# distributed-lab/era-boojum

Hardware: AMD Instinct MI355X
Metric: LDE+Merkle commit Goldilocks elems/s (2^22x256, LDE x4) (higher is better)
Workload: dtype u64 (Goldilocks); 1 GPU; C3: 2^22 rows x 256 cols, LDE x4, Poseidon2 cap 16; rows=4194304, cols=256, lde=4, cap=16, tree_hasher=poseidon2, parallelism=single, launch=stream

## Files before the change

### era-boojum_amd/csrc/merkle.hip

```cpp
#include <hip/hip_runtime.h>
#include "gl.hpp"
#include "poseidon2.hpp"
#include "poseidon2_quad.hpp"
#include "bj_internal.hpp"
#include "tree_hasher.hpp"

namespace bj {

constexpr int LEAF_THREADS = 256;

__device__ __forceinline__ void store_canon4(const p2::State& s, uint64_t* o) {
    uint32_t z0[4], z1[4];
    glasm::canon_x4(s.lo[0], s.hi[0], z0[0], z1[0], s.lo[1], s.hi[1], z0[1], z1[1],
                    s.lo[2], s.hi[2], z0[2], z1[2], s.lo[3], s.hi[3], z0[3], z1[3]);
#pragma unroll
    for (int i = 0; i < 4; i++) o[i] = ((uint64_t)z1[i] << 32) | z0[i];
}

__device__ __forceinline__ void store_canon4_at(const p2::State& s, int q, uint64_t* o) {
    const int b = 4 * q;
    uint32_t z0[4], z1[4];
    glasm::canon_x4(s.lo[b], s.hi[b], z0[0], z1[0], s.lo[b + 1], s.hi[b + 1], z0[1], z1[1],
                    s.lo[b + 2], s.hi[b + 2], z0[2], z1[2], s.lo[b + 3], s.hi[b + 3], z0[3], z1[3]);
#pragma unroll
    for (int i = 0; i < 4; i++) o[i] = ((uint64_t)z1[i] << 32) | z0[i];
}

__device__ __forceinline__ void load8(p2::State& s, const uint64_t* q, size_t stride, uint32_t count) {
#pragma unroll
    for (int i = 0; i < 8; i++) {
        uint64_t v = (uint32_t)i < count ? q[(size_t)i * stride] : 0;
        s.lo[i] = (uint32_t)v;
        s.hi[i] = (uint32_t)(v >> 32);
    }
}

template <bool HAS_IN, bool FINAL, bool REM>
__device__ __forceinline__ void leaf_hash_body(const uint64_t* __restrict__ src, size_t col_stride, uint32_t n_cols,
                                               size_t n_leaves, const uint64_t* cap_in, uint64_t* out) {
    const size_t L = blockIdx.x * (size_t)LEAF_THREADS + threadIdx.x;
    if (L >= n_leaves) return;
    const uint64_t* p = src + L;
    p2::State s;
#pragma unroll
    for (int i = 0; i < 12; i++) s.lo[i] = s.hi[i] = 0;
    if (HAS_IN) {
#pragma unroll
        for (int i = 0; i < 4; i++) {
            const uint64_t v = cap_in[4 * L + i];
            s.lo[8 + i] = (uint32_t)v;
            s.hi[8 + i] = (uint32_t)(v >> 32);
        }
    }
    const uint32_t full = n_cols >> 3;
    const uint32_t rem = REM ? n_cols & 7 : 0;
    uint64_t nxt[8];
    if (full > 0) {
#pragma unroll
        for (int i = 0; i < 8; i++) nxt[i] = p[(size_t)i * col_stride];
    }
    if (full > 0) {
        for (uint32_t g = 0; g + 1 < full; g++) {
#pragma unroll
            for (int i = 0; i < 8; i++) {
                s.lo[i] = (uint32_t)nxt[i];
                s.hi[i] = (uint32_t)(nxt[i] >> 32);
            }
            const uint64_t* q = p + (size_t)(g + 1) * 8 * col_stride;
#pragma unroll
            for (int i = 0; i < 8; i++) nxt[i] = q[(size_t)i * col_stride];
            p2::permute<p2::OUT_CAP>(s);
        }
#pragma unroll
        for (int i = 0; i < 8; i++) {
            s.lo[i] = (uint32_t)nxt[i];
            s.hi[i] = (uint32_t)(nxt[i] >> 32);
        }
        if (FINAL && !REM)
            p2::permute<p2::OUT_DIGEST>(s);
        else
            p2::permute<p2::OUT_CAP>(s);
    }
    if (FINAL && REM) {
        load8(s, p + (size_t)full * 8 * col_stride, col_stride, rem);
        p2::permute<p2::OUT_DIGEST>(s);
    }
    if (FINAL) store_canon4(s, out + 4 * L);
    else store_canon4_at(s, 2, out + 4 * L);
}

template <bool HAS_IN, bool FINAL, bool REM>
__global__ __launch_bounds__(LEAF_THREADS) void leaf_hash_kernel(const uint64_t* __restrict__ src,
                                                                 size_t col_stride, uint32_t n_cols,
                                                                 size_t n_leaves, const uint64_t* cap_in,
                                                                 uint64_t* out) {
    leaf_hash_body<HAS_IN, FINAL, REM>(src, col_stride, n_cols, n_leaves, cap_in, out);
}

__global__ __launch_bounds__(LEAF_THREADS) void leaf_chunk_kernel(const uint64_t* __restrict__ src,
                                                                  size_t col_stride, uint32_t n_cols,
                                                                  uint32_t log_e, size_t n_leaves,
                                                                  uint64_t* __restrict__ out) {
    const size_t L = blockIdx.x * (size_t)LEAF_THREADS + threadIdx.x;
    if (L >= n_leaves) return;
    const uint32_t E = 1u << log_e;
    const uint64_t* p = src + (L << log_e);
    p2::State s;
#pragma unroll
    for (int i = 0; i < 12; i++) s.lo[i] = s.hi[i] = 0;
    const uint32_t total = n_cols << log_e;
    uint32_t k = 0;
    for (; k + 8 < total; k += 8) {
#pragma unroll
        for (int i = 0; i < 8; i++) {
            const uint32_t e = k + i;
            const uint64_t v = p[(size_t)(e >> log_e) * col_stride + (e & (E - 1))];
            s.lo[i] = (uint32_t)v;
            s.hi[i] = (uint32_t)(v >> 32);
        }
        p2::permute<p2::OUT_CAP>(s);
    }
    if (k < total) {
#pragma unroll
        for (int i = 0; i < 8; i++) {
            const uint32_t e = k + i;
            const uint64_t v = e < total ? p[(size_t)(e >> log_e) * col_stride + (e & (E - 1))] : 0;
            s.lo[i] = (uint32_t)v;
            s.hi[i] = (uint32_t)(v >> 32);
        }
        p2::permute<p2::OUT_DIGEST>(s);
    }
    store_canon4(s, out + 4 * L);
}

struct P2Node {
    static __device__ __forceinline__ void node(const uint64_t* l, const uint64_t* r, uint64_t* o) {
        p2::State s;
#pragma unroll
        for (int i = 0; i < 4; i++) {
            s.lo[i] = (uint32_t)l[i];
            s.hi[i] = (uint32_t)(l[i] >> 32);
            s.lo[4 + i] = (uint32_t)r[i];
            s.hi[4 + i] = (uint32_t)(r[i] >> 32);
            s.lo[8 + i] = s.hi[8 + i] = 0;
        }
        p2::permute<p2::OUT_DIGEST>(s);
        store_canon4(s, o);
    }
};

__global__ __launch_bounds__(256) void node_level_q4_kernel(const uint64_t* __restrict__ prev,
                                                            uint64_t* __restrict__ next, size_t m) {
    __shared__ uint64_t rcf[8 * 12];
    const uint32_t t = threadIdx.x;
    if (t < 8 * 12) {
        const uint32_t r = t / 12, e = t % 12, row = r < 4 ? r : r + 22;
        rcf[t] = p2::RCL.lo[row][e] | (p2::RCL.hi[row][e] << 32);
    }
    __syncthreads();
    const size_t i = (blockIdx.x * (size_t)256 + t) >> 2;
    const uint32_t p = t & 3;
    if (i >= m) return;
    const p2q::Consts k = p2q::consts(p);
    const uint64_t l = prev[8 * i + p], r = prev[8 * i + 4 + p];
    uint32_t lo[3] = {(uint32_t)l, (uint32_t)r, 0}, hi[3] = {(uint32_t)(l >> 32), (uint32_t)(r >> 32), 0};
    p2q::permute(lo, hi, rcf, p, k);
    uint32_t z0, z1;
    glasm::canon_x1(lo[0], hi[0], z0, z1);
    next[4 * i + p] = ((uint64_t)z1 << 32) | z0;
}

constexpr uint32_t NODE_FUSED_THREADS = 512;
constexpr uint32_t NODE_FUSED_LOG_DIGESTS = 8;
__global__ __launch_bounds__(NODE_FUSED_THREADS) void node_levels_q4_kernel(const uint64_t* __restrict__ prev,
                                                                           uint64_t* __restrict__ out, size_t len,
                                                                           uint32_t b, uint32_t lv) {
    __shared__ uint64_t rcf[8 * 12];
    __shared__ uint64_t buf[2][(NODE_FUSED_THREADS / 4) * 4];
    const uint32_t t = threadIdx.x;
    if (t < 8 * 12) {
        const uint32_t r = t / 12, e = t % 12, row = r < 4 ? r : r + 22;
        rcf[t] = p2::RCL.lo[row][e] | (p2::RCL.hi[row][e] << 32);
    }
    __syncthreads();
    const uint32_t q = t >> 2, p = t & 3;
    const p2q::Consts k = p2q::consts(p);
    size_t base = 0, level_len = len >> 1;
    uint32_t nodes = 1u << (b - 1);
    for (uint32_t j = 0; j < lv; j++) {
        if (q < nodes) {
            uint64_t l, r;
            if (j == 0) {
                const size_t i = (size_t)blockIdx.x * nodes + q;
                l = prev[8 * i + p];
                r = prev[8 * i + 4 + p];
            } else {
                l = buf[(j - 1) & 1][8 * q + p];
                r = buf[(j - 1) & 1][8 * q + 4 + p];
            }
            uint32_t lo[3] = {(uint32_t)l, (uint32_t)r, 0}, hi[3] = {(uint32_t)(l >> 32), (uint32_t)(r >> 32), 0};
            p2q::permute(lo, hi, rcf, p, k);
            uint32_t z0, z1;
            glasm::canon_x1(lo[0], hi[0], z0, z1);
            const uint64_t z = ((uint64_t)z1 << 32) | z0;
            out[4 * (base + (size_t)blockIdx.x * nodes + q) + p] = z;
            buf[j & 1][4 * q + p] = z;
        }
        __syncthreads();
        base += level_len;
        level_len >>= 1;
        nodes >>= 1;
    }
}

__global__ __launch_bounds__(256) void permute_kernel(uint64_t* states, size_t count) {
    const size_t i = blockIdx.x * (size_t)256 + threadIdx.x;
    if (i >= count) return;
    p2::State s;
#pragma unroll
    for (int k = 0; k < 12; k++) {
        uint64_t v = states[12 * i + k];
        s.lo[k] = (uint32_t)v;
        s.hi[k] = (uint32_t)(v >> 32);
    }
    p2::permute(s);
#pragma unroll
    for (int q = 0; q < 3; q++) store_canon4_at(s, q, states + 12 * i + 4 * q);
}

hipError_t launch_leaves(const uint64_t* src, size_t col_stride, uint32_t n_cols, size_t n_leaves, uint64_t* out,
                         hipStream_t st) {
    return launch_leaves_partial(src, col_stride, n_cols, n_leaves, nullptr, out, true, st);
}

hipError_t launch_leaves_partial(const uint64_t* src, size_t col_stride, uint32_t n_cols, size_t n_leaves,
                                 const uint64_t* cap_in, uint64_t* out, bool final_, hipStream_t st) {
    if (n_leaves == 0) return hipSuccess;
    const dim3 g((unsigned)((n_leaves + LEAF_THREADS - 1) / LEAF_THREADS));
#define BJ_LEAF(IN, FIN, REM) \
    hipLaunchKernelGGL((leaf_hash_kernel<IN, FIN, REM>), g, dim3(LEAF_THREADS), 0, st, src, col_stride, n_cols, \
                       n_leaves, cap_in, out)
#define BJ_LEAF_R(IN, FIN) \
    do {                     \
        if (n_cols & 7)      \
            BJ_LEAF(IN, FIN, true); \
        else                 \
            BJ_LEAF(IN, FIN, false); \
    } while (0)
    if (cap_in) {
        if (final_) BJ_LEAF_R(true, true);
        else BJ_LEAF_R(true, false);
    } else {
        if (final_) BJ_LEAF_R(false, true);
        else BJ_LEAF_R(false, false);
    }
#undef BJ_LEAF_R
#undef BJ_LEAF
    return hipGetLastError();
}

hipError_t launch_leaves_chunked(const uint64_t* src, size_t col_stride, uint32_t n_cols, uint32_t log_e,
                                 size_t n_leaves, uint64_t* out, hipStream_t st) {
    if (n_leaves == 0) return hipSuccess;
    hipLaunchKernelGGL(leaf_chunk_kernel, dim3((unsigned)((n_leaves + LEAF_THREADS - 1) / LEAF_THREADS)),
                       dim3(LEAF_THREADS), 0, st, src, col_stride, n_cols, log_e, n_leaves, out);
    return hipGetLastError();
}

static size_t node_q4_max() { return (size_t)knobs().node_q4_max; }

hipError_t launch_nodes(const uint64_t* leaves, size_t n_leaves, uint32_t cap_size, uint64_t* nodes,
                        hipStream_t st) {
    const size_t q4max = node_q4_max();
    if (!q4max) return launch_nodes_per_lane<P2Node>(leaves, n_leaves, cap_size, nodes, 512, st);
    const uint64_t* prev = leaves;
    uint64_t* out = nodes;
    size_t len = n_leaves;
    const auto pow2 = [](size_t x) { return x && !(x & (x - 1)); };
    const bool fuse = knobs().node_fused && pow2(n_leaves) && pow2(cap_size);
    while (len > cap_size) {
        size_t m = len / 2;
        if (m <= q4max && fuse) {
            uint32_t L = 0, C = 0;
            while (((size_t)1 << L) < len) L++;
            while (((size_t)1 << C) < cap_size) C++;
            const uint32_t b = std::min(NODE_FUSED_LOG_DIGESTS, L), lv = std::min(b, L - C);
            hipLaunchKernelGGL(node_levels_q4_kernel, dim3((unsigned)(len >> b)), dim3(NODE_FUSED_THREADS), 0, st,
                               prev, out, len, b, lv);
            prev = out + 4 * (len - (len >> (lv - 1)));
            out += 4 * (len - (len >> lv));
            len >>= lv;
            continue;
        }
        if (m <= q4max)
            hipLaunchKernelGGL(node_level_q4_kernel, dim3((unsigned)((m + 63) / 64)), dim3(256), 0, st, prev, out, m);
        else
            hipLaunchKernelGGL(node_level_kernel<P2Node>, dim3((unsigned)((m + 255) / 256)), dim3(256), 0, st, prev,
                               out, m);
        prev = out;
        out += 4 * m;
        len = m;
    }
    return hipGetLastError();
}

hipError_t launch_permute(uint64_t* states, size_t count, hipStream_t st) {
    if (count == 0) return hipSuccess;
    hipLaunchKernelGGL(permute_kernel, dim3((unsigned)((count + 255) / 256)), dim3(256), 0, st, states, count);
    return hipGetLastError();
}

}
```

### era-boojum_amd/csrc/poseidon2.hpp

```cpp
#pragma once
#include "gl.hpp"
#include "gl_asm.hpp"

namespace p2 {

struct RcLimbs {
    uint64_t lo[30][12];
    uint64_t hi[30][12];
};

constexpr uint64_t RC_FLAT[30][12] = {
#include "poseidon2_rc.inc"
};

constexpr RcLimbs make_rc_limbs() {
    RcLimbs r{};
    for (int i = 0; i < 30; i++)
        for (int j = 0; j < 12; j++) {
            r.lo[i][j] = RC_FLAT[i][j] & 0xFFFFFFFFull;
            r.hi[i][j] = RC_FLAT[i][j] >> 32;
        }
    return r;
}

__device__ __constant__ static const RcLimbs RCL = make_rc_limbs();

namespace sched {
constexpr uint64_t P = 0xFFFFFFFF00000001ull;
constexpr uint64_t addm(uint64_t a, uint64_t b) { return (uint64_t)(((unsigned __int128)a + b) % P); }
constexpr uint64_t subm(uint64_t a, uint64_t b) { return addm(a, P - b % P); }
constexpr uint64_t mulm(uint64_t a, uint64_t b) { return (uint64_t)(((unsigned __int128)a * b) % P); }
constexpr int SH[12] = {4, 14, 11, 8, 0, 5, 2, 9, 13, 6, 3, 12};
constexpr uint64_t FULL_RC_BOUND = ~0ull - (1ull << 41) + 1;
constexpr uint64_t LIMB_RC_BOUND = (1ull << 63) + (1ull << 62);
struct Values {
    uint64_t k[11];
    uint64_t d[10];
    uint64_t rc26[12];
};
constexpr Values derive() {
    Values v{};
    uint64_t f[12] = {RC_FLAT[4][0]};
    for (int q = 0; q < 11; q++) {
        const int r = 4 + 2 * q;
        uint64_t s = 0;
        for (int i = 1; i < 12; i++) s = addm(s, f[i]);
        v.k[q] = subm(RC_FLAT[r + 1][0], s);
        f[0] = 0;
        for (int i = 0; i < 12; i++) f[i] = addm(addm(mulm(f[i], 1ull << SH[i]), s), v.k[q]);
        s = 0;
        for (int i = 1; i < 12; i++) s = addm(s, f[i]);
        f[0] = 0;
        for (int i = 0; i < 12; i++) f[i] = addm(mulm(f[i], 1ull << SH[i]), s);
        if (q < 10) {
            v.d[q] = subm(RC_FLAT[r + 2][0], f[0]);
            f[0] = RC_FLAT[r + 2][0];
        }
    }
    for (int i = 0; i < 12; i++) v.rc26[i] = subm(RC_FLAT[26][i], f[i]);
    return v;
}
constexpr Values V = derive();
constexpr bool full_rcs_fit() {
    for (int r : {0, 1, 2, 3, 27, 28, 29})
        for (int i = 0; i < 12; i++)
            if (RC_FLAT[r][i] >= FULL_RC_BOUND) return false;
    return RC_FLAT[4][0] < FULL_RC_BOUND;
}
static_assert(full_rcs_fit(), "a full-round constant is too large for the one-add form");

constexpr uint64_t LAZY_OFF = 2 * 0xFFFFFFFFull;
constexpr uint64_t me_row_sum(int i) { return (i & 1) ? 48 : 64; }
constexpr uint64_t lazy_off(int i) { return me_row_sum(i) * LAZY_OFF; }
constexpr uint64_t lazy_fix_lo(int i) { return 1 + 2 * me_row_sum(i); }
constexpr uint64_t lazy_fix_hi(int i) { return 0xFFFFFFFFull - 2 * me_row_sum(i); }
constexpr bool lazy_in(int r) { return (r >= 1 && r <= 3) || (r >= 27 && r <= 29); }
constexpr bool lazy_rcs_fit() {
    for (int r = 0; r < 30; r++)
        for (int i = 0; i < 12; i++)
            if ((lazy_in(r) || (r == 4 && i == 0)) &&
                (RC_FLAT[r][i] < lazy_off(i) || RC_FLAT[r][i] - lazy_off(i) >= FULL_RC_BOUND))
                return false;
    return true;
}
static_assert(lazy_rcs_fit(), "a full-round constant is smaller than the lazy offset it takes out");
static_assert((lazy_fix_lo(0) + (lazy_fix_hi(0) << 32) + lazy_off(0)) == P &&
                  (lazy_fix_lo(1) + (lazy_fix_hi(1) << 32) + lazy_off(1)) == P,
              "the two-limb form of -lazy_off");
}

struct Sched {
    uint64_t rcw8[30][8];
    uint64_t rcw4[30][4];
    uint64_t k_lo[11], k_hi[11];
    uint64_t d_lo[10], d_hi[10];
    uint64_t rc26_w[12], rc26_lo[12], rc26_hi[12];
    uint64_t rcl8[30][8];
    uint64_t rcl4[30][4];
};
constexpr Sched make_sched() {
    Sched s{};
    for (int r = 0; r < 30; r++)
        for (int i = 0; i < 12; i++) {
            (i < 8 ? s.rcw8[r][i] : s.rcw4[r][i - 8]) = RC_FLAT[r][i];
            const bool lazy = sched::lazy_in(r) || (r == 4 && i == 0);
            (i < 8 ? s.rcl8[r][i] : s.rcl4[r][i - 8]) = RC_FLAT[r][i] - (lazy ? sched::lazy_off(i) : 0);
        }
    for (int q = 0; q < 11; q++) { s.k_lo[q] = sched::V.k[q] & 0xFFFFFFFFull; s.k_hi[q] = sched::V.k[q] >> 32; }
    for (int q = 0; q < 10; q++) { s.d_lo[q] = sched::V.d[q] & 0xFFFFFFFFull; s.d_hi[q] = sched::V.d[q] >> 32; }
    for (int i = 0; i < 12; i++) {
        s.rc26_w[i] = sched::V.rc26[i];
        s.rc26_lo[i] = sched::V.rc26[i] & 0xFFFFFFFFull;
        s.rc26_hi[i] = sched::V.rc26[i] >> 32;
    }
    return s;
}
__device__ __constant__ static const Sched SCH = make_sched();

struct State {
    uint32_t lo[12], hi[12];
};

__device__ __forceinline__ void sbox_lazy_x4(const uint32_t* lo, const uint32_t* hi, uint64_t* Lin, uint64_t* Hin) {
    uint32_t a0, a1, b0, b1, c0, c1, d0, d1;
    glasm::mul_x4(lo[0], hi[0], lo[0], hi[0], a0, a1, lo[1], hi[1], lo[1], hi[1], b0, b1,
                  lo[2], hi[2], lo[2], hi[2], c0, c1, lo[3], hi[3], lo[3], hi[3], d0, d1);
    uint32_t e0, e1, f0, f1, g0, g1, h0, h1;
    glasm::mul_x4(a0, a1, lo[0], hi[0], e0, e1, b0, b1, lo[1], hi[1], f0, f1,
                  c0, c1, lo[2], hi[2], g0, g1, d0, d1, lo[3], hi[3], h0, h1);
    uint32_t i0, i1, j0, j1, k0, k1, l0, l1;
    glasm::mul_x4(a0, a1, a0, a1, i0, i1, b0, b1, b0, b1, j0, j1,
                  c0, c1, c0, c1, k0, k1, d0, d1, d0, d1, l0, l1);
    glasm::mul_lazy_x4(e0, e1, i0, i1, Lin[0], Hin[0], f0, f1, j0, j1, Lin[1], Hin[1],
                       g0, g1, k0, k1, Lin[2], Hin[2], h0, h1, l0, l1, Lin[3], Hin[3]);
}

__device__ __forceinline__ void sbox_x1(uint32_t& lo, uint32_t& hi) {
    uint32_t a0, a1, e0, e1, i0, i1;
    glasm::mul_x1(lo, hi, lo, hi, a0, a1);
    glasm::mul_x2(a0, a1, lo, hi, e0, e1, a0, a1, a0, a1, i0, i1);
    glasm::mul_x1(e0, e1, i0, i1, lo, hi);
}

__device__ __forceinline__ void m4_limbs(uint64_t& x0, uint64_t& x1, uint64_t& x2, uint64_t& x3) {
    uint64_t t0 = x0 + x1;
    uint64_t t1 = x2 + x3;
    uint64_t t2 = (x1 << 1) + t1;
    uint64_t t3 = (x3 << 1) + t0;
    uint64_t t4 = (t1 << 2) + t3;
    uint64_t t5 = (t0 << 2) + t2;
    uint64_t t6 = t3 + t5;
    uint64_t t7 = t2 + t4;
    x0 = t6; x1 = t5; x2 = t7; x3 = t4;
}

__device__ __forceinline__ uint64_t add_lo_u64(uint32_t lo, uint64_t b) {
    uint64_t r;
    asm volatile("v_mad_u64_u32 %0, vcc, %1, 1, %2" : "=v"(r) : "v"(lo), "s"(b) : "vcc");
    return r;
}

enum Out { OUT_ALL = 0, OUT_CAP = 1, OUT_DIGEST = 2 };

template <int OUT = OUT_ALL>
__device__ __forceinline__ void mds_ext_limbs(uint64_t* X) {
    m4_limbs(X[0], X[1], X[2], X[3]);
    m4_limbs(X[4], X[5], X[6], X[7]);
    m4_limbs(X[8], X[9], X[10], X[11]);
#pragma unroll
    for (int i = 0; i < 4; i++) {
        uint64_t a = X[i], b = X[i + 4], c = X[i + 8];
        if constexpr (OUT == OUT_ALL) {
            uint64_t s = a + b + c;
            X[i] = s + a;
            X[i + 4] = s + b;
            X[i + 8] = s + c;
        } else if constexpr (OUT == OUT_CAP) {
            X[i + 8] = (c << 1) + a + b;
        } else {
            X[i] = (a << 1) + b + c;
        }
    }
}

template <int OUT = OUT_ALL>
__device__ __forceinline__ void mds_ext_limbs(const uint32_t* v, uint64_t* X) {
#pragma unroll
    for (int i = 0; i < 12; i++) X[i] = v[i];
    mds_ext_limbs<OUT>(X);
}

__device__ __forceinline__ void split(uint64_t z, uint32_t& lo, uint32_t& hi) {
    lo = (uint32_t)z;
    hi = (uint32_t)(z >> 32);
}

template <int OUT = OUT_ALL>
__device__ __forceinline__ void reduce12(const uint64_t* L, const uint64_t* H, uint32_t* lo, uint32_t* hi) {
#pragma unroll
    for (int q = 0; q < 3; q++) {
        if constexpr (OUT == OUT_CAP) { if (q != 2) continue; }
        if constexpr (OUT == OUT_DIGEST) { if (q != 0) continue; }
        const int i = 4 * q;
        uint64_t z[4];
        glasm::reduce_x4(L[i], (uint32_t)H[i], (uint32_t)(H[i] >> 32), z[0],
                         L[i + 1], (uint32_t)H[i + 1], (uint32_t)(H[i + 1] >> 32), z[1],
                         L[i + 2], (uint32_t)H[i + 2], (uint32_t)(H[i + 2] >> 32), z[2],
                         L[i + 3], (uint32_t)H[i + 3], (uint32_t)(H[i + 3] >> 32), z[3]);
#pragma unroll
        for (int j = 0; j < 4; j++) split(z[j], lo[i + j], hi[i + j]);
    }
}

template <int OUT = OUT_ALL, bool RC = true>
__device__ __forceinline__ void full_round(State& s, uint64_t* L, uint64_t* H, int r) {
    if constexpr (RC) {
#pragma unroll
        for (int i = 0; i < 12; i++) L[i] += i < 8 ? SCH.rcl8[r][i] : SCH.rcl4[r][i - 8];
    }
    reduce12(L, H, s.lo, s.hi);
#pragma unroll
    for (int q = 0; q < 3; q++) sbox_lazy_x4(s.lo + 4 * q, s.hi + 4 * q, L + 4 * q, H + 4 * q);
    mds_ext_limbs<OUT>(L);
    mds_ext_limbs<OUT>(H);
}

template <int I>
__device__ __forceinline__ void lazy_fix(uint64_t* L, uint64_t* H) {
    L[I] += sched::lazy_fix_lo(I);
    H[I] += sched::lazy_fix_hi(I);
}
template <int I, int N>
__device__ __forceinline__ void lazy_fix_range(uint64_t* L, uint64_t* H) {
    lazy_fix<I>(L, H);
    if constexpr (I + 1 < N) lazy_fix_range<I + 1, N>(L, H);
}

struct Partial {
    uint64_t z0;
    uint64_t W[12];
    uint32_t G[12];
};

template <bool HALF>
__device__ __forceinline__ void partial_first(const Partial& P, int q, uint64_t* L, uint64_t* H, uint32_t& lo0,
                                              uint32_t& hi0) {
    uint64_t z0;
    uint32_t lo[12], hi[12];
    const uint64_t kl = SCH.k_lo[q], kh = SCH.k_hi[q];
    split(P.z0, lo[0], hi[0]);
#pragma unroll
    for (int i = 1; i < 12; i++) split(P.W[i], lo[i], hi[i]);
    sbox_x1(lo[0], hi[0]);
    if constexpr (HALF) glasm::mi_layer_a_g(lo, hi, P.G, kl, kh, L, H, z0);
    else glasm::mi_layer_a(lo, hi, kl, kh, L, H, z0);
    split(z0, lo0, hi0);
    sbox_x1(lo0, hi0);
}

template <bool HALF>
__device__ __forceinline__ void partial_round_pair(Partial& P, int q) {
    uint64_t L[12], H[12], Lo[12], Ho[12];
    uint32_t lo0, hi0, hh[12];
    const uint64_t dl = SCH.d_lo[q], dh = SCH.d_hi[q];
    partial_first<HALF>(P, q, L, H, lo0, hi0);
    glasm::mi_layer_b_half(lo0, hi0, L, H, dl, dh, Lo, Ho, P.z0);
#pragma unroll
    for (int i = 1; i < 12; i++) split(Ho[i], P.G[i], hh[i]);
    glasm::eps_fold_x11(hh, Lo, P.W);
}

__device__ __forceinline__ void partial_round_pair_last(const Partial& P, uint64_t* Lo, uint64_t* Ho) {
    uint64_t L[12], H[12];
    uint32_t lo0, hi0;
    partial_first<true>(P, 10, L, H, lo0, hi0);
    glasm::mi_layer_b_limbs(lo0, hi0, L, H, Lo, Ho);
}

template <int I = 0>
__device__ __forceinline__ void add_rc26(uint64_t* L, uint64_t* H) {
    if constexpr (sched::V.rc26[I] < sched::LIMB_RC_BOUND) {
        L[I] += SCH.rc26_w[I];
    } else {
        L[I] += SCH.rc26_lo[I];
        H[I] += SCH.rc26_hi[I];
    }
    if constexpr (I + 1 < 12) add_rc26<I + 1>(L, H);
}

template <int OUT = OUT_ALL>
__device__ __forceinline__ void permute(State& s) {
    uint64_t L[12], H[12], Z[12];
    Partial P;
    mds_ext_limbs(s.lo, L);
    mds_ext_limbs(s.hi, H);
#pragma unroll 1
    for (int r = 0; r < 4; r++) full_round(s, L, H, r);
    L[0] += SCH.rcl8[4][0];
    lazy_fix_range<1, 12>(L, H);
#pragma unroll
    for (int q = 0; q < 3; q++) {
        const int i = 4 * q;
        glasm::reduce_x4(L[i], (uint32_t)H[i], (uint32_t)(H[i] >> 32), Z[i],
                         L[i + 1], (uint32_t)H[i + 1], (uint32_t)(H[i + 1] >> 32), Z[i + 1],
                         L[i + 2], (uint32_t)H[i + 2], (uint32_t)(H[i + 2] >> 32), Z[i + 2],
                         L[i + 3], (uint32_t)H[i + 3], (uint32_t)(H[i + 3] >> 32), Z[i + 3]);
    }
    P.z0 = Z[0];
#pragma unroll
    for (int i = 1; i < 12; i++) P.W[i] = Z[i];
    partial_round_pair<false>(P, 0);
#pragma unroll 1
    for (int q = 1; q < 10; q++) partial_round_pair<true>(P, q);
    partial_round_pair_last(P, L, H);
    add_rc26(L, H);
    full_round<OUT_ALL, false>(s, L, H, 26);
#pragma unroll 1
    for (int r = 27; r < 29; r++) full_round(s, L, H, r);
    full_round<OUT>(s, L, H, 29);
    if constexpr (OUT == OUT_ALL) lazy_fix_range<0, 12>(L, H);
    else if constexpr (OUT == OUT_CAP) lazy_fix_range<8, 12>(L, H);
    else lazy_fix_range<0, 4>(L, H);
    reduce12<OUT>(L, H, s.lo, s.hi);
}

__device__ __forceinline__ void permute(uint64_t v[12]) {
    State s;
#pragma unroll
    for (int i = 0; i < 12; i++) {
        s.lo[i] = (uint32_t)v[i];
        s.hi[i] = (uint32_t)(v[i] >> 32);
    }
    permute(s);
#pragma unroll
    for (int i = 0; i < 12; i++) v[i] = ((uint64_t)s.hi[i] << 32) | s.lo[i];
}

}
```

Before: 5.891 billion elems/s.

## Carry unreduced capacity limbs between sponge permutations in leaf hashing

Leaf hashing now keeps the four capacity words in lazy two-limb form across sponge absorptions instead of fully reducing them after each permutation. The lazy offset is folded into modified round-0 constants through the external MDS. A second change replaces the first partial round's full reduce_x4 entry with a single reduce plus an epsilon fold, so all partial round pairs share one path. This removes per-permutation reduction work on the capacity lanes, at the cost of extra constant tables and tighter bound reasoning, which is checked by static_asserts.

```diff
diff --git a/era-boojum_amd/csrc/merkle.hip b/era-boojum_amd/csrc/merkle.hip
--- a/era-boojum_amd/csrc/merkle.hip
+++ b/era-boojum_amd/csrc/merkle.hip
@@ -52,6 +52,8 @@
             s.hi[8 + i] = (uint32_t)(v >> 32);
         }
     }
+    p2::CapLimbs cap;
+    p2::cap_limbs_from_words(s.lo, s.hi, cap);
     const uint32_t full = n_cols >> 3;
     const uint32_t rem = REM ? n_cols & 7 : 0;
     uint64_t nxt[8];
@@ -69,7 +71,7 @@
             const uint64_t* q = p + (size_t)(g + 1) * 8 * col_stride;
 #pragma unroll
             for (int i = 0; i < 8; i++) nxt[i] = q[(size_t)i * col_stride];
-            p2::permute<p2::OUT_CAP>(s);
+            p2::permute_cap_limbs<p2::OUT_CAP_LIMBS>(s, cap);
         }
 #pragma unroll
         for (int i = 0; i < 8; i++) {
@@ -77,13 +79,15 @@
             s.hi[i] = (uint32_t)(nxt[i] >> 32);
         }
         if (FINAL && !REM)
-            p2::permute<p2::OUT_DIGEST>(s);
+            p2::permute_cap_limbs<p2::OUT_DIGEST>(s, cap);
+        else if (FINAL)
+            p2::permute_cap_limbs<p2::OUT_CAP_LIMBS>(s, cap);
         else
-            p2::permute<p2::OUT_CAP>(s);
+            p2::permute_cap_limbs<p2::OUT_CAP>(s, cap);
     }
     if (FINAL && REM) {
         load8(s, p + (size_t)full * 8 * col_stride, col_stride, rem);
-        p2::permute<p2::OUT_DIGEST>(s);
+        p2::permute_cap_limbs<p2::OUT_DIGEST>(s, cap);
     }
     if (FINAL) store_canon4(s, out + 4 * L);
     else store_canon4_at(s, 2, out + 4 * L);
@@ -109,6 +113,8 @@
 #pragma unroll
     for (int i = 0; i < 12; i++) s.lo[i] = s.hi[i] = 0;
     const uint32_t total = n_cols << log_e;
+    p2::CapLimbs cap;
+    p2::cap_limbs_from_words(s.lo, s.hi, cap);
     uint32_t k = 0;
     for (; k + 8 < total; k += 8) {
 #pragma unroll
@@ -118,7 +124,7 @@
             s.lo[i] = (uint32_t)v;
             s.hi[i] = (uint32_t)(v >> 32);
         }
-        p2::permute<p2::OUT_CAP>(s);
+        p2::permute_cap_limbs<p2::OUT_CAP_LIMBS>(s, cap);
     }
     if (k < total) {
 #pragma unroll
@@ -128,7 +134,7 @@
             s.lo[i] = (uint32_t)v;
             s.hi[i] = (uint32_t)(v >> 32);
         }
-        p2::permute<p2::OUT_DIGEST>(s);
+        p2::permute_cap_limbs<p2::OUT_DIGEST>(s, cap);
     }
     store_canon4(s, out + 4 * L);
 }
diff --git a/era-boojum_amd/csrc/poseidon2.hpp b/era-boojum_amd/csrc/poseidon2.hpp
--- a/era-boojum_amd/csrc/poseidon2.hpp
+++ b/era-boojum_amd/csrc/poseidon2.hpp
@@ -87,6 +87,38 @@
 static_assert((lazy_fix_lo(0) + (lazy_fix_hi(0) << 32) + lazy_off(0)) == P &&
                   (lazy_fix_lo(1) + (lazy_fix_hi(1) << 32) + lazy_off(1)) == P,
               "the two-limb form of -lazy_off");
+
+constexpr uint64_t LIMB_IN_RC_BOUND = ~0ull - (1ull << 47) + 1;
+constexpr void m4_const(uint64_t* x) {
+    const uint64_t t0 = x[0] + x[1], t1 = x[2] + x[3];
+    const uint64_t t2 = (x[1] << 1) + t1, t3 = (x[3] << 1) + t0;
+    const uint64_t t4 = (t1 << 2) + t3, t5 = (t0 << 2) + t2;
+    x[0] = t3 + t5; x[1] = t5; x[2] = t2 + t4; x[3] = t4;
+}
+struct Off12 {
+    uint64_t v[12];
+};
+constexpr Off12 limb_in_offsets() {
+    Off12 o{};
+    for (int i = 8; i < 12; i++) o.v[i] = lazy_off(i);
+    for (int b = 0; b < 12; b += 4) m4_const(o.v + b);
+    for (int i = 0; i < 4; i++) {
+        const uint64_t s = o.v[i] + o.v[i + 4] + o.v[i + 8];
+        o.v[i] += s; o.v[i + 4] += s; o.v[i + 8] += s;
+    }
+    return o;
+}
+constexpr Off12 LIMB_IN_OFF = limb_in_offsets();
+constexpr bool limb_in_fits(int i) {
+    return RC_FLAT[0][i] >= LIMB_IN_OFF.v[i] && RC_FLAT[0][i] - LIMB_IN_OFF.v[i] < LIMB_IN_RC_BOUND;
+}
+constexpr uint64_t limb_in_rc(int i) { return RC_FLAT[0][i] - (limb_in_fits(i) ? LIMB_IN_OFF.v[i] : 0); }
+constexpr bool limb_in_ok() {
+    for (int i = 0; i < 12; i++)
+        if (LIMB_IN_OFF.v[i] >= (1ull << 45) || limb_in_rc(i) >= LIMB_IN_RC_BOUND) return false;
+    return true;
+}
+static_assert(limb_in_ok(), "a limb-entry round-0 constant is negative or too large for the one-add form");
 }
 
 struct Sched {
@@ -117,6 +149,20 @@
 }
 __device__ __constant__ static const Sched SCH = make_sched();
 
+struct LimbIn {
+    uint64_t rc8[4][8];
+    uint64_t rc4[4][4];
+};
+constexpr LimbIn make_limb_in() {
+    LimbIn t{};
+    for (int r = 0; r < 4; r++)
+        for (int i = 0; i < 12; i++)
+            (i < 8 ? t.rc8[r][i] : t.rc4[r][i - 8]) =
+                r == 0 ? sched::limb_in_rc(i) : RC_FLAT[r][i] - sched::lazy_off(i);
+    return t;
+}
+__device__ __constant__ static const LimbIn LIMBIN = make_limb_in();
+
 struct State {
     uint32_t lo[12], hi[12];
 };
@@ -160,7 +206,19 @@
     return r;
 }
 
-enum Out { OUT_ALL = 0, OUT_CAP = 1, OUT_DIGEST = 2 };
+enum Out { OUT_ALL = 0, OUT_CAP = 1, OUT_DIGEST = 2, OUT_CAP_LIMBS = 3 };
+
+struct CapLimbs {
+    uint64_t L[4], H[4];
+};
+
+__device__ __forceinline__ void cap_limbs_from_words(const uint32_t* lo, const uint32_t* hi, CapLimbs& c) {
+#pragma unroll
+    for (int j = 0; j < 4; j++) {
+        c.L[j] = lo[8 + j] + sched::lazy_off(8 + j);
+        c.H[j] = hi[8 + j];
+    }
+}
 
 template <int OUT = OUT_ALL>
 __device__ __forceinline__ void mds_ext_limbs(uint64_t* X) {
@@ -175,7 +233,7 @@
             X[i] = s + a;
             X[i + 4] = s + b;
             X[i + 8] = s + c;
-        } else if constexpr (OUT == OUT_CAP) {
+        } else if constexpr (OUT == OUT_CAP || OUT == OUT_CAP_LIMBS) {
             X[i + 8] = (c << 1) + a + b;
         } else {
             X[i] = (a << 1) + b + c;
@@ -190,6 +248,14 @@
     mds_ext_limbs<OUT>(X);
 }
 
+__device__ __forceinline__ void mds_ext_limbs_in(const uint32_t* v, const uint64_t* cap, uint64_t* X) {
+#pragma unroll
+    for (int i = 0; i < 8; i++) X[i] = v[i];
+#pragma unroll
+    for (int j = 0; j < 4; j++) X[8 + j] = cap[j];
+    mds_ext_limbs(X);
+}
+
 __device__ __forceinline__ void split(uint64_t z, uint32_t& lo, uint32_t& hi) {
     lo = (uint32_t)z;
     hi = (uint32_t)(z >> 32);
@@ -200,6 +266,7 @@
 #pragma unroll
     for (int q = 0; q < 3; q++) {
         if constexpr (OUT == OUT_CAP) { if (q != 2) continue; }
+        static_assert(OUT != OUT_CAP_LIMBS, "the limb form of the capacity words is not reduced");
         if constexpr (OUT == OUT_DIGEST) { if (q != 0) continue; }
         const int i = 4 * q;
         uint64_t z[4];
@@ -212,9 +279,12 @@
     }
 }
 
-template <int OUT = OUT_ALL, bool RC = true>
+template <int OUT = OUT_ALL, bool RC = true, bool LIMB_IN = false>
 __device__ __forceinline__ void full_round(State& s, uint64_t* L, uint64_t* H, int r) {
-    if constexpr (RC) {
+    if constexpr (RC && LIMB_IN) {
+#pragma unroll
+        for (int i = 0; i < 12; i++) L[i] += i < 8 ? LIMBIN.rc8[r][i] : LIMBIN.rc4[r][i - 8];
+    } else if constexpr (RC) {
 #pragma unroll
         for (int i = 0; i < 12; i++) L[i] += i < 8 ? SCH.rcl8[r][i] : SCH.rcl4[r][i - 8];
     }
@@ -236,13 +306,21 @@
     if constexpr (I + 1 < N) lazy_fix_range<I + 1, N>(L, H);
 }
 
+template <int I = 0>
+__device__ __forceinline__ void limb_in_fix(uint64_t* L, uint64_t* H) {
+    if constexpr (!sched::limb_in_fits(I)) {
+        L[I] += (sched::P - sched::LIMB_IN_OFF.v[I]) & 0xFFFFFFFFull;
+        H[I] += (sched::P - sched::LIMB_IN_OFF.v[I]) >> 32;
+    }
+    if constexpr (I + 1 < 12) limb_in_fix<I + 1>(L, H);
+}
+
 struct Partial {
     uint64_t z0;
     uint64_t W[12];
     uint32_t G[12];
 };
 
-template <bool HALF>
 __device__ __forceinline__ void partial_first(const Partial& P, int q, uint64_t* L, uint64_t* H, uint32_t& lo0,
                                               uint32_t& hi0) {
     uint64_t z0;
@@ -252,18 +330,16 @@
 #pragma unroll
     for (int i = 1; i < 12; i++) split(P.W[i], lo[i], hi[i]);
     sbox_x1(lo[0], hi[0]);
-    if constexpr (HALF) glasm::mi_layer_a_g(lo, hi, P.G, kl, kh, L, H, z0);
-    else glasm::mi_layer_a(lo, hi, kl, kh, L, H, z0);
+    glasm::mi_layer_a_g(lo, hi, P.G, kl, kh, L, H, z0);
     split(z0, lo0, hi0);
     sbox_x1(lo0, hi0);
 }
 
-template <bool HALF>
 __device__ __forceinline__ void partial_round_pair(Partial& P, int q) {
     uint64_t L[12], H[12], Lo[12], Ho[12];
     uint32_t lo0, hi0, hh[12];
     const uint64_t dl = SCH.d_lo[q], dh = SCH.d_hi[q];
-    partial_first<HALF>(P, q, L, H, lo0, hi0);
+    partial_first(P, q, L, H, lo0, hi0);
     glasm::mi_layer_b_half(lo0, hi0, L, H, dl, dh, Lo, Ho, P.z0);
 #pragma unroll
     for (int i = 1; i < 12; i++) split(Ho[i], P.G[i], hh[i]);
@@ -273,7 +349,7 @@
 __device__ __forceinline__ void partial_round_pair_last(const Partial& P, uint64_t* Lo, uint64_t* Ho) {
     uint64_t L[12], H[12];
     uint32_t lo0, hi0;
-    partial_first<true>(P, 10, L, H, lo0, hi0);
+    partial_first(P, 10, L, H, lo0, hi0);
     glasm::mi_layer_b_limbs(lo0, hi0, L, H, Lo, Ho);
 }
 
@@ -288,40 +364,61 @@
     if constexpr (I + 1 < 12) add_rc26<I + 1>(L, H);
 }
 
-template <int OUT = OUT_ALL>
-__device__ __forceinline__ void permute(State& s) {
-    uint64_t L[12], H[12], Z[12];
+template <int OUT, bool LIMB_IN>
+__device__ __forceinline__ void permute_form(State& s, CapLimbs& cap) {
+    uint64_t L[12], H[12];
     Partial P;
-    mds_ext_limbs(s.lo, L);
-    mds_ext_limbs(s.hi, H);
+    if constexpr (LIMB_IN) {
+        mds_ext_limbs_in(s.lo, cap.L, L);
+        mds_ext_limbs_in(s.hi, cap.H, H);
+        limb_in_fix(L, H);
+    } else {
+        mds_ext_limbs(s.lo, L);
+        mds_ext_limbs(s.hi, H);
+    }
 #pragma unroll 1
-    for (int r = 0; r < 4; r++) full_round(s, L, H, r);
+    for (int r = 0; r < 4; r++) full_round<OUT_ALL, true, LIMB_IN>(s, L, H, r);
     L[0] += SCH.rcl8[4][0];
     lazy_fix_range<1, 12>(L, H);
-#pragma unroll
-    for (int q = 0; q < 3; q++) {
-        const int i = 4 * q;
-        glasm::reduce_x4(L[i], (uint32_t)H[i], (uint32_t)(H[i] >> 32), Z[i],
-                         L[i + 1], (uint32_t)H[i + 1], (uint32_t)(H[i + 1] >> 32), Z[i + 1],
-                         L[i + 2], (uint32_t)H[i + 2], (uint32_t)(H[i + 2] >> 32), Z[i + 2],
-                         L[i + 3], (uint32_t)H[i + 3], (uint32_t)(H[i + 3] >> 32), Z[i + 3]);
-    }
-    P.z0 = Z[0];
-#pragma unroll
-    for (int i = 1; i < 12; i++) P.W[i] = Z[i];
-    partial_round_pair<false>(P, 0);
+    glasm::reduce_x1(L[0], (uint32_t)H[0], (uint32_t)(H[0] >> 32), P.z0);
+    {
+        uint32_t hh[12];
+#pragma unroll
+        for (int i = 1; i < 12; i++) split(H[i], P.G[i], hh[i]);
+        glasm::eps_fold_x11(hh, L, P.W);
+    }
 #pragma unroll 1
-    for (int q = 1; q < 10; q++) partial_round_pair<true>(P, q);
+    for (int q = 0; q < 10; q++) partial_round_pair(P, q);
     partial_round_pair_last(P, L, H);
     add_rc26(L, H);
     full_round<OUT_ALL, false>(s, L, H, 26);
 #pragma unroll 1
     for (int r = 27; r < 29; r++) full_round(s, L, H, r);
     full_round<OUT>(s, L, H, 29);
-    if constexpr (OUT == OUT_ALL) lazy_fix_range<0, 12>(L, H);
-    else if constexpr (OUT == OUT_CAP) lazy_fix_range<8, 12>(L, H);
-    else lazy_fix_range<0, 4>(L, H);
-    reduce12<OUT>(L, H, s.lo, s.hi);
+    if constexpr (OUT == OUT_CAP_LIMBS) {
+#pragma unroll
+        for (int j = 0; j < 4; j++) {
+            cap.L[j] = L[8 + j];
+            cap.H[j] = H[8 + j];
+        }
+    } else {
+        if constexpr (OUT == OUT_ALL) lazy_fix_range<0, 12>(L, H);
+        else if constexpr (OUT == OUT_CAP) lazy_fix_range<8, 12>(L, H);
+        else lazy_fix_range<0, 4>(L, H);
+        reduce12<OUT>(L, H, s.lo, s.hi);
+    }
+}
+
+template <int OUT = OUT_ALL>
+__device__ __forceinline__ void permute(State& s) {
+    static_assert(OUT != OUT_CAP_LIMBS, "the limb form needs a CapLimbs");
+    CapLimbs none;
+    permute_form<OUT, false>(s, none);
+}
+
+template <int OUT>
+__device__ __forceinline__ void permute_cap_limbs(State& s, CapLimbs& cap) {
+    permute_form<OUT, true>(s, cap);
 }
 
 __device__ __forceinline__ void permute(uint64_t v[12]) {
```

Measured after the change: 5.914 billion elems/s (median of 6 runs). Within noise of the previous version (+0.4%).
